# bramtoula/multi_robot_SLAM_separators

Hardware: AMD Instinct MI355X
Metric: candidate keyframe-pair verifications/sec (NetVLAD NN + ORB match + RANSAC) @1/2/4/8 GPU (higher is better)
Workload: dtype u8+f16+f32+f64

## Files before the change

multi_robot_slam_separators_amd/csrc/k_match.hip:

```cpp
#include "sf_internal.hpp"
#include <type_traits>

namespace {

__device__ __forceinline__ uint32_t bcnt_acc(uint32_t x, uint32_t acc) {
  uint32_t r;
  asm("v_bcnt_u32_b32 %0, %1, %2" : "=v"(r) : "v"(x), "v"(acc));
  return r;
}

template <int W, int NQ>
__device__ __forceinline__ void knn2_scan(const uint32_t* __restrict__ dF, int Kf, const uint32_t (&q)[NQ][W],
                                          uint32_t (&k1)[NQ], uint32_t (&k2)[NQ]) {
#pragma unroll 4
  for (int f = 0; f < Kf; ++f) {
    const uint32_t* r = dF + (size_t)f * W;
    uint32_t x[W];
#pragma unroll
    for (int c = 0; c < W; ++c) x[c] = r[c];
#pragma unroll
    for (int j = 0; j < NQ; ++j) {
      uint32_t d = 0;
#pragma unroll
      for (int c = 0; c < W; ++c) d = bcnt_acc(x[c] ^ q[j][c], d);
      const uint32_t key = (d << 16) | (uint32_t)f;
      k2[j] = min(max(key, k1[j]), k2[j]);
      k1[j] = min(k1[j], key);
    }
  }
}

template <int W>
__device__ __forceinline__ void knn2_scan_l2(const uint32_t* __restrict__ dF, int Kf, const uint32_t (&q)[W], float& d1,
                                             float& d2, int& i1) {
#pragma unroll 1
  for (int f = 0; f < Kf; ++f) {
    const uint32_t* r = dF + (size_t)f * W;
    float s = 0.f;
#pragma unroll
    for (int c = 0; c < W; ++c) {
      const float d = __uint_as_float(q[c]) - __uint_as_float(r[c]);
      s = s + d * d;
    }
    if (s < d1) { d2 = d1; d1 = s; i1 = f; }
    else if (s < d2) { d2 = s; }
  }
}

template <int W>
__device__ __forceinline__ void knn2_scan_l2_halves(const uint32_t* __restrict__ dF, int Kf,
                                                    const uint32_t* __restrict__ qrow, float& d1, float& d2, int& i1) {
  static_assert(W == 128, "two halves of 64 dimensions");
  constexpr int H = 64, FB = 16;
#pragma unroll 1
  for (int f0 = 0; f0 < Kf; f0 += FB) {
    float s[FB];
#pragma unroll
    for (int j = 0; j < FB; ++j) s[j] = 0.f;
#pragma unroll 1
    for (int half = 0; half < 2; ++half) {
      uint32_t q[H];
      {
        const uint4* p = reinterpret_cast<const uint4*>(qrow + half * H);
#pragma unroll
        for (int c = 0; c < H / 4; ++c) {
          const uint4 v = p[c];
          q[4 * c] = v.x; q[4 * c + 1] = v.y; q[4 * c + 2] = v.z; q[4 * c + 3] = v.w;
        }
      }
#pragma unroll
      for (int j = 0; j < FB; ++j) {
        if (f0 + j < Kf) {
          const uint32_t* r = dF + (size_t)(f0 + j) * W + half * H;
          float a = s[j];
#pragma unroll
          for (int c = 0; c < H; ++c) {
            const float d = __uint_as_float(q[c]) - __uint_as_float(r[c]);
            a = a + d * d;
          }
          s[j] = a;
        }
      }
    }
#pragma unroll
    for (int j = 0; j < FB; ++j) {
      if (f0 + j < Kf) {
        if (s[j] < d1) { d2 = d1; d1 = s[j]; i1 = f0 + j; }
        else if (s[j] < d2) { d2 = s[j]; }
      }
    }
  }
}

template <int W>
__device__ __forceinline__ void load_desc(const uint32_t* __restrict__ base, int row, bool valid, uint32_t (&q)[W]) {
  const uint4* p = reinterpret_cast<const uint4*>(base + (size_t)(valid ? row : 0) * W);
#pragma unroll
  for (int c = 0; c < W / 4; ++c) {
    uint4 v = p[c];
    q[4 * c + 0] = v.x; q[4 * c + 1] = v.y; q[4 * c + 2] = v.z; q[4 * c + 3] = v.w;
  }
}

template <int W, int NQ, int NT, bool L2 = false>
__global__ void __launch_bounds__(NT)
k_match_global(StoreView st, const int32_t* __restrict__ pair_from, const int32_t* __restrict__ pair_to,
               float nndr, int min_inliers, int est, uint32_t* __restrict__ corr, CorrHeader* __restrict__ hdr,
               PassState* __restrict__ pass, int32_t* __restrict__ list, int32_t* __restrict__ counter) {
  extern __shared__ __attribute__((aligned(16))) int smem[];
  constexpr int NW = NT / 64;
  const int pair = blockIdx.x;
  const int tid = threadIdx.x;
  const int lane = tid & 63, wave = tid >> 6;
  const int kcap = st.kcap;
  const int sF = pair_from[pair], sT = pair_to[pair];
  if ((unsigned)sF >= (unsigned)st.n_slots || (unsigned)sT >= (unsigned)st.n_slots) {
    if (tid == 0) {
      CorrHeader h = {0, 0, 0, 0};
      hdr[pair] = h;
      PassState ps;
#pragma unroll
      for (int i = 0; i < 12; ++i) ps.T[i] = 0.f;
      ps.var = 1.0; ps.var_ang = 1.0; ps.is_null = 1; ps.inliers = 0; ps.matches = 0; ps.pad = 0;
      pass[pair] = ps;
    }
    return;
  }
  const int4 mF = st.meta[sF], mT = st.meta[sT];
  const int Kf = mF.x, Kt = mT.x;
  const uint32_t* dF = st.desc + (size_t)sF * kcap * W;
  const uint32_t* dT = st.desc + (size_t)sT * kcap * W;

  int* cnt = smem;
  int* owner = smem + kcap;
  int* misc = smem + 2 * kcap;

  for (int i = tid; i < Kf; i += NT) cnt[i] = 0;
  if (tid < 16) misc[tid] = 0;
  __syncthreads();

  int rejected = 0;
  if constexpr (L2) {
    static_assert(!L2 || NQ == 1, "one resident float row per lane");
    if (Kf > 0) {
      for (int base = 0; base < Kt; base += NT) {
        const int t = base + tid;
        float d1 = __int_as_float(0x7F800000), d2 = __int_as_float(0x7F800000);
        int i1 = -1;
        if constexpr (W > 64) {
          if (Kt - base - (tid & ~63) > 0)
            knn2_scan_l2_halves<W>(dF, Kf, dT + (size_t)(t < Kt ? t : 0) * W, d1, d2, i1);
        } else {
          uint32_t q[W];
          load_desc<W>(dT, t, t < Kt, q);
          if (Kt - base - (tid & ~63) > 0)
            knn2_scan_l2<W>(dF, Kf, q, d1, d2, i1);
        }
        if (t < Kt) {
          const bool acc = (Kf >= 2) && i1 >= 0 && !(d1 > nndr * d2);
          if (acc) {
            atomicAdd(&cnt[i1], 1);
            owner[i1] = t;
          } else {
            ++rejected;
          }
        }
      }
    }
  } else
  if (Kf > 0) {
    for (int base = 0; base < Kt; base += NQ * NT) {
      uint32_t q[NQ][W], k1[NQ], k2[NQ];
#pragma unroll
      for (int j = 0; j < NQ; ++j) {
        const int t = base + j * NT + tid;
        load_desc<W>(dT, t, t < Kt, q[j]);
        k1[j] = 0xFFFFFFFFu;
        k2[j] = 0xFFFFFFFFu;
      }
      const int wave_rows = Kt - base - (tid & ~63);
      const int groups = wave_rows <= 0 ? 0 : min(NQ, (wave_rows + NT - 1) / NT);
      if (groups == NQ) {
        knn2_scan<W, NQ>(dF, Kf, q, k1, k2);
      } else if (groups > 0) {
#pragma unroll
        for (int j = 0; j < NQ; ++j) {
          if (j < groups) {
            uint32_t qq[1][W], a1[1] = {0xFFFFFFFFu}, a2[1] = {0xFFFFFFFFu};
#pragma unroll
            for (int c = 0; c < W; ++c) qq[0][c] = q[j][c];
            knn2_scan<W, 1>(dF, Kf, qq, a1, a2);
            k1[j] = a1[0];
            k2[j] = a2[0];
          }
        }
      }
#pragma unroll
      for (int j = 0; j < NQ; ++j) {
        const int t = base + j * NT + tid;
        if (t < Kt) {
          const bool acc = (Kf >= 2) && !((float)(k1[j] >> 16) > nndr * (float)(k2[j] >> 16));
          if (acc) {
            const int f = (int)(k1[j] & 0xFFFFu);
            atomicAdd(&cnt[f], 1);
            owner[f] = t;
          } else {
            ++rejected;
          }
        }
      }
    }
  }
  for (int off = 32; off >= 1; off >>= 1) rejected += __shfl_xor(rejected, off);
  if (lane == 0 && rejected) atomicAdd(&misc[0], rejected);
  __syncthreads();

  uint32_t* out = corr + (size_t)pair * kcap;
  int running = 0;
  for (int base = 0; base < Kf; base += NT) {
    const int f = base + tid;
    const bool flag = (f < Kf) && (cnt[f] == 1);
    const unsigned long long bal = __ballot(flag);
    const int before = __popcll(bal & ((1ull << lane) - 1ull));
    if (lane == 0) misc[4 + wave] = __popcll(bal);
    __syncthreads();
    int woff = 0, total = 0;
#pragma unroll
    for (int w = 0; w < NW; ++w) {
      int c = misc[4 + w];
      if (w < wave) woff += c;
      total += c;
    }
    if (flag) out[running + woff + before] = (uint32_t)f | ((uint32_t)owner[f] << 16);
    running += total;
    __syncthreads();
  }
  const int n_corr = running;

  const int unique_to = (Kf > 0 && Kt > 0) ? misc[0] + n_corr : 0;
  const int words_from = (Kf > 0 && mF.y > 0) ? Kf : 0;
  const int words_to = (mT.y > 0) ? unique_to : 0;
  const bool motion = est == 0 ? (unique_to > 0 && words_from >= min_inliers && words_to >= min_inliers)
                    : est == 1 ? (unique_to > 0 && words_from >= min_inliers && unique_to >= min_inliers)
                               : (est == 3 && unique_to > 0 && ((words_from >= min_inliers && unique_to >= min_inliers) ||
                                                                (words_to >= min_inliers && Kf >= min_inliers)));
  const bool survivor = est == 3 ? (motion && n_corr > 0) : (motion && n_corr >= min_inliers && n_corr >= (est == 0 ? 3 : 4));
  if (motion && !survivor) {
    const float* xF = st.xyz + (size_t)sF * kcap * 3;
    const float* xT = st.xyz + (size_t)sT * kcap * 3;
    for (int i = tid; i < n_corr; i += NT) {
      uint32_t c = out[i];
      const float* a = xF + 3 * (c & 0xFFFFu);
      const float* b = xT + 3 * (c >> 16);
      bool ok = isfinite(a[0]) && isfinite(a[1]) && isfinite(a[2]);
      if (est == 0)
        ok = ok && isfinite(b[0]) && isfinite(b[1]) && isfinite(b[2]) && (a[0] != 0.f || a[1] != 0.f || a[2] != 0.f) &&
             (b[0] != 0.f || b[1] != 0.f || b[2] != 0.f);
      if (ok) atomicAdd(&misc[2], 1);
    }
    __syncthreads();
  }
  if (tid == 0) {
    CorrHeader h;
    h.n_corr = n_corr;
    h.words_from = words_from;
    h.words_to = words_to;
    h.words_to_2d = unique_to;
    hdr[pair] = h;
    PassState ps;
#pragma unroll
    for (int i = 0; i < 12; ++i) ps.T[i] = 0.f;
    ps.var = 1.0; ps.var_ang = 1.0;
    ps.is_null = 1;
    ps.inliers = 0;
    ps.matches = (motion && !survivor) ? misc[2] : 0;
    ps.pad = 0;
    pass[pair] = ps;
    if (survivor) {
      int pos = atomicAdd(counter, 1);
      list[pos] = pair;
    }
  }
}

__device__ __forceinline__ uint32_t min_u16(uint32_t a, uint32_t b) {
  uint32_t r;
  asm("v_min_u16 %0, %1, %2" : "=v"(r) : "v"(a), "v"(b));
  return r;
}
__device__ __forceinline__ uint32_t max_u16(uint32_t a, uint32_t b) {
  uint32_t r;
  asm("v_max_u16 %0, %1, %2" : "=v"(r) : "v"(a), "v"(b));
  return r;
}

constexpr int MATCH_CH = 16;

template <int W, int NQ>
__device__ __forceinline__ void knn2_step_lds(const uint32_t* fromD, int f, const uint32_t (&q)[NQ][W],
                                              uint32_t (&d1)[NQ], uint32_t (&d2)[NQ]) {
  const uint4* r = reinterpret_cast<const uint4*>(fromD + (size_t)f * W);
  uint32_t x[W];
#pragma unroll
  for (int c = 0; c < W / 4; ++c) {
    const uint4 v = r[c];
    x[4 * c] = v.x; x[4 * c + 1] = v.y; x[4 * c + 2] = v.z; x[4 * c + 3] = v.w;
  }
#pragma unroll
  for (int j = 0; j < NQ; ++j) {
    uint32_t d = 0;
#pragma unroll
    for (int c = 0; c < W; ++c) d = bcnt_acc(x[c] ^ q[j][c], d);
    d2[j] = min_u16(d2[j], max_u16(d, d1[j]));
    d1[j] = min_u16(d1[j], d);
  }
}

template <int W, int NQ>
__device__ __forceinline__ void knn2_scan_lds(const uint32_t* fromD, int Kf, const uint32_t (&q)[NQ][W],
                                              uint32_t (&d1)[NQ], uint32_t (&d2)[NQ], uint32_t (&chunk)[NQ]) {
  int c0 = 0;
  for (; c0 + MATCH_CH <= Kf; c0 += MATCH_CH) {
    uint32_t prev[NQ];
#pragma unroll
    for (int j = 0; j < NQ; ++j) prev[j] = d1[j];
#pragma unroll 4
    for (int u = 0; u < MATCH_CH; ++u) knn2_step_lds<W, NQ>(fromD, c0 + u, q, d1, d2);
#pragma unroll
    for (int j = 0; j < NQ; ++j) chunk[j] = ((d1[j] & 0xFFFFu) != (prev[j] & 0xFFFFu)) ? (uint32_t)c0 : chunk[j];
  }
  if (c0 < Kf) {
    uint32_t prev[NQ];
#pragma unroll
    for (int j = 0; j < NQ; ++j) prev[j] = d1[j];
    for (int f = c0; f < Kf; ++f) knn2_step_lds<W, NQ>(fromD, f, q, d1, d2);
#pragma unroll
    for (int j = 0; j < NQ; ++j) chunk[j] = ((d1[j] & 0xFFFFu) != (prev[j] & 0xFFFFu)) ? (uint32_t)c0 : chunk[j];
  }
}

typedef int mf_v8i __attribute__((ext_vector_type(8)));
typedef float mf_v16f __attribute__((ext_vector_type(16)));
constexpr float MF_FR = 1.f / 2048.f;
constexpr int MF_MAX_ROWS = 2048;

__device__ __forceinline__ mf_v8i fp4_spread_from(uint32_t x, uint32_t m88, uint32_t c22) {
  mf_v8i o = {0, 0, 0, 0, 0, 0, 0, 0};
  o[0] = (int)((x & m88) | c22);
  o[1] = (int)(x & 0x44444444u);
  o[2] = (int)(x & 0x22222222u);
  o[3] = (int)(x & 0x11111111u);
  return o;
}
__device__ __forceinline__ mf_v8i fp4_spread_to(uint32_t y, uint32_t m88, uint32_t c22) {
  mf_v8i o = {0, 0, 0, 0, 0, 0, 0, 0};
  const uint32_t n = ~y;
  o[0] = (int)((y & m88) | c22);
  o[1] = (int)(((n << 1) & m88) | c22);
  o[2] = (int)(((n << 2) & m88) | 0x44444444u);
  o[3] = (int)(((n << 3) & m88) | 0x66666666u);
  return o;
}

static inline size_t sf_match_lds_bytes(int kcap, int w) {
  const int behind = 2 * kcap + 16;
  return (size_t)(kcap * w + (behind > 32 * w ? behind : 32 * w)) * sizeof(int);
}

template <int KS>
__device__ __forceinline__ void load_raw(const uint32_t* p, uint32_t (&raw)[KS]) {
#pragma unroll
  for (int c = 0; c < KS / 4; ++c) {
    const uint4 v = reinterpret_cast<const uint4*>(p)[c];
    raw[4 * c] = v.x; raw[4 * c + 1] = v.y; raw[4 * c + 2] = v.z; raw[4 * c + 3] = v.w;
  }
}

__device__ __forceinline__ void top2_update16(const mf_v16f& v, float& b, float& s) {
  const float x0 = __builtin_amdgcn_fmed3f(b, v[0], v[1]);
  float ta, tb;
  asm("v_max3_f32 %0, %0, %4, %5\n\t"
      "v_med3_f32 %2, %0, %6, %7\n\t"
      "v_max3_f32 %0, %0, %6, %7\n\t"
      "v_max3_f32 %1, %1, %20, %2\n\t"
      "v_med3_f32 %2, %0, %8, %9\n\t"
      "v_max3_f32 %0, %0, %8, %9\n\t"
      "v_med3_f32 %3, %0, %10, %11\n\t"
      "v_max3_f32 %0, %0, %10, %11\n\t"
      "v_max3_f32 %1, %1, %2, %3\n\t"
      "v_med3_f32 %2, %0, %12, %13\n\t"
      "v_max3_f32 %0, %0, %12, %13\n\t"
      "v_med3_f32 %3, %0, %14, %15\n\t"
      "v_max3_f32 %0, %0, %14, %15\n\t"
      "v_max3_f32 %1, %1, %2, %3\n\t"
      "v_med3_f32 %2, %0, %16, %17\n\t"
      "v_max3_f32 %0, %0, %16, %17\n\t"
      "v_med3_f32 %3, %0, %18, %19\n\t"
      "v_max3_f32 %0, %0, %18, %19\n\t"
      "v_max3_f32 %1, %1, %2, %3"
      : "+v"(b), "+v"(s), "=&v"(ta), "=&v"(tb)
      : "v"(v[0]), "v"(v[1]), "v"(v[2]), "v"(v[3]), "v"(v[4]), "v"(v[5]), "v"(v[6]), "v"(v[7]), "v"(v[8]), "v"(v[9]),
        "v"(v[10]), "v"(v[11]), "v"(v[12]), "v"(v[13]), "v"(v[14]), "v"(v[15]), "v"(x0));
}

template <int W, int NTL, bool TAIL>
__device__ __forceinline__ void knn2_mfma_tile(const uint32_t* fromD, int Kf, int mt, int r, int h,
                                               const mf_v8i (&Bf)[NTL][W / 2], const float (&cin)[16],
                                               float (&b)[NTL], float (&s)[NTL], uint32_t m88, uint32_t c22,
                                               uint32_t (&raw)[W / 2], const uint32_t*& nxt) {
  constexpr int KS = W / 2;
  mf_v16f c0;
#pragma unroll
  for (int i = 0; i < 16; ++i) c0[i] = cin[i];
  mf_v8i Af[KS];
#pragma unroll
  for (int k = 0; k < KS; ++k) Af[k] = fp4_spread_from(raw[k], m88, c22);
  if (!TAIL) {
    nxt += 32 * W;
    load_raw<KS>(nxt, raw);
  }
#pragma unroll
  for (int j = 0; j < NTL; ++j) {
    b[j] += 32.f * MF_FR;
    s[j] += 32.f * MF_FR;
  }
#pragma unroll
  for (int j = 0; j < NTL; ++j) {
    mf_v16f acc = __builtin_amdgcn_mfma_scale_f32_32x32x64_f8f6f4(Af[0], Bf[j][0], c0, 4, 4, 0, 0, 0, 0);
#pragma unroll
    for (int k = 1; k < KS; ++k)
      acc = __builtin_amdgcn_mfma_scale_f32_32x32x64_f8f6f4(Af[k], Bf[j][k], acc, 4, 4, 0, 0, 0, 0);
    if (TAIL) {
      const int left = Kf - mt * 32 - 4 * h;
#pragma unroll
      for (int i = 0; i < 16; ++i) acc[i] = ((i & 3) + 8 * (i >> 2) < left) ? acc[i] : -INFINITY;
    }
    top2_update16(acc, b[j], s[j]);
  }
}

template <int W, int NTL>
struct MfB {
  mf_v8i Bf[NTL][W / 2];
  int tsum[NTL];
};

template <int W, int NTL>
__device__ __forceinline__ void mf_load_b(const uint32_t* __restrict__ dT, int Kt, const int (&tile)[NTL], int lane,
                                          MfB<W, NTL>& B) {
  constexpr int KS = W / 2;
  const int r = lane & 31, h = lane >> 5;
  uint32_t m88, c22;
  asm volatile("v_mov_b32 %0, 0x88888888" : "=v"(m88));
  asm volatile("v_mov_b32 %0, 0x22222222" : "=v"(c22));
#pragma unroll
  for (int j = 0; j < NTL; ++j) {
    const int t = tile[j] * 32 + r;
    uint32_t raw[KS];
#pragma unroll
    for (int k = 0; k < KS; ++k) raw[k] = 0;
    if (t < Kt) load_raw<KS>(dT + (size_t)t * W + KS * h, raw);
    int p = 0;
#pragma unroll
    for (int k = 0; k < KS; ++k) {
      B.Bf[j][k] = fp4_spread_to(raw[k], m88, c22);
      p += __popc(raw[k] & 0x77777777u);
    }
    p += __shfl_xor(p, 32);
    B.tsum[j] = 24 * W - 2 * p;
  }
}

typedef int mf_v4i __attribute__((ext_vector_type(4)));

__device__ __forceinline__ void mf_pipe_half1(mf_v16f& acc, const mf_v4i& a0, const mf_v4i& a1, const mf_v4i& a2,
                                              const mf_v4i& a3, const mf_v4i& b0, const mf_v4i& b1, const mf_v16f& cin,
                                              const mf_v16f& old, float& b, float& s, float& x0, float& ta, float& tb) {
  asm volatile(
      "s_nop 1\n\t"
      "v_mfma_f32_32x32x64_f8f6f4 %[acc], %[a0], %[b0], %[cin] cbsz:4 blgp:4\n\t"
      "v_add_f32 %[b], 0x3c800000, %[b]\n\t"
      "v_add_f32 %[s], 0x3c800000, %[s]\n\t"
      "s_nop 1\n\t"
      "v_med3_f32 %[x0], %[b], %[o0], %[o1]\n\t"
      "v_max3_f32 %[b], %[b], %[o0], %[o1]\n\t"
      "v_mfma_f32_32x32x64_f8f6f4 %[acc], %[a1], %[b1], %[acc] cbsz:4 blgp:4\n\t"
      "v_med3_f32 %[ta], %[b], %[o2], %[o3]\n\t"
      "v_max3_f32 %[b], %[b], %[o2], %[o3]\n\t"
      "v_max3_f32 %[s], %[s], %[x0], %[ta]\n\t"
      "v_med3_f32 %[ta], %[b], %[o4], %[o5]\n\t"
      "v_max3_f32 %[b], %[b], %[o4], %[o5]\n\t"
      "v_med3_f32 %[tb], %[b], %[o6], %[o7]"
      : [acc] "=&v"(acc), [b] "+v"(b), [s] "+v"(s), [x0] "=&v"(x0), [ta] "=&v"(ta), [tb] "=&v"(tb)
      : [a0] "v"(a0), [a1] "v"(a1), "v"(a2), "v"(a3), [b0] "v"(b0), [b1] "v"(b1), [cin] "v"(cin), [o0] "v"(old[0]),
        [o1] "v"(old[1]), [o2] "v"(old[2]), [o3] "v"(old[3]), [o4] "v"(old[4]), [o5] "v"(old[5]), [o6] "v"(old[6]),
        [o7] "v"(old[7]));
}
__device__ __forceinline__ void mf_pipe_half2(mf_v16f& acc, const mf_v4i& a2, const mf_v4i& a3, const mf_v4i& b2,
                                              const mf_v4i& b3, const mf_v16f& old, float& b, float& s, float& ta,
                                              float& tb) {
  float x0;
  asm volatile(
      "v_mfma_f32_32x32x64_f8f6f4 %[acc], %[a2], %[b2], %[acc] cbsz:4 blgp:4\n\t"
      "v_max3_f32 %[b], %[b], %[o6], %[o7]\n\t"
      "v_max3_f32 %[s], %[s], %[ta], %[tb]\n\t"
      "v_med3_f32 %[x0], %[b], %[o8], %[o9]\n\t"
      "v_max3_f32 %[b], %[b], %[o8], %[o9]\n\t"
      "v_med3_f32 %[ta], %[b], %[o10], %[o11]\n\t"
      "v_max3_f32 %[b], %[b], %[o10], %[o11]\n\t"
      "v_mfma_f32_32x32x64_f8f6f4 %[acc], %[a3], %[b3], %[acc] cbsz:4 blgp:4\n\t"
      "v_max3_f32 %[s], %[s], %[x0], %[ta]\n\t"
      "v_med3_f32 %[ta], %[b], %[o12], %[o13]\n\t"
      "v_max3_f32 %[b], %[b], %[o12], %[o13]\n\t"
      "v_med3_f32 %[tb], %[b], %[o14], %[o15]\n\t"
      "v_max3_f32 %[b], %[b], %[o14], %[o15]\n\t"
      "v_max3_f32 %[s], %[s], %[ta], %[tb]"
      : [acc] "+v"(acc), [b] "+v"(b), [s] "+v"(s), [x0] "=&v"(x0), [ta] "+v"(ta), [tb] "+v"(tb)
      : [a2] "v"(a2), [a3] "v"(a3), [b2] "v"(b2), [b3] "v"(b3), [o6] "v"(old[6]), [o7] "v"(old[7]), [o8] "v"(old[8]),
        [o9] "v"(old[9]), [o10] "v"(old[10]), [o11] "v"(old[11]), [o12] "v"(old[12]), [o13] "v"(old[13]),
        [o14] "v"(old[14]), [o15] "v"(old[15]));
}
__device__ __forceinline__ void mf_pipe_drain(const mf_v16f& old, float& b, float& s) {
  float x0, ta, tb;
  asm volatile(
      "s_nop 11\n\t"
      "v_add_f32 %[b], 0x3c800000, %[b]\n\t"
      "v_add_f32 %[s], 0x3c800000, %[s]\n\t"
      "v_med3_f32 %[x0], %[b], %[o0], %[o1]\n\t"
      "v_max3_f32 %[b], %[b], %[o0], %[o1]\n\t"
      "v_med3_f32 %[ta], %[b], %[o2], %[o3]\n\t"
      "v_max3_f32 %[b], %[b], %[o2], %[o3]\n\t"
      "v_max3_f32 %[s], %[s], %[x0], %[ta]\n\t"
      "v_med3_f32 %[ta], %[b], %[o4], %[o5]\n\t"
      "v_max3_f32 %[b], %[b], %[o4], %[o5]\n\t"
      "v_med3_f32 %[tb], %[b], %[o6], %[o7]\n\t"
      "v_max3_f32 %[b], %[b], %[o6], %[o7]\n\t"
      "v_max3_f32 %[s], %[s], %[ta], %[tb]\n\t"
      "v_med3_f32 %[x0], %[b], %[o8], %[o9]\n\t"
      "v_max3_f32 %[b], %[b], %[o8], %[o9]\n\t"
      "v_med3_f32 %[ta], %[b], %[o10], %[o11]\n\t"
      "v_max3_f32 %[b], %[b], %[o10], %[o11]\n\t"
      "v_max3_f32 %[s], %[s], %[x0], %[ta]\n\t"
      "v_med3_f32 %[ta], %[b], %[o12], %[o13]\n\t"
      "v_max3_f32 %[b], %[b], %[o12], %[o13]\n\t"
      "v_med3_f32 %[tb], %[b], %[o14], %[o15]\n\t"
      "v_max3_f32 %[b], %[b], %[o14], %[o15]\n\t"
      "v_max3_f32 %[s], %[s], %[ta], %[tb]"
      : [b] "+v"(b), [s] "+v"(s), [x0] "=&v"(x0), [ta] "=&v"(ta), [tb] "=&v"(tb)
      : [o0] "v"(old[0]), [o1] "v"(old[1]), [o2] "v"(old[2]), [o3] "v"(old[3]), [o4] "v"(old[4]), [o5] "v"(old[5]),
        [o6] "v"(old[6]), [o7] "v"(old[7]), [o8] "v"(old[8]), [o9] "v"(old[9]), [o10] "v"(old[10]), [o11] "v"(old[11]),
        [o12] "v"(old[12]), [o13] "v"(old[13]), [o14] "v"(old[14]), [o15] "v"(old[15]));
}

template <int NTL>
__device__ __forceinline__ void mf_scan_full_tiles_pipe(const uint32_t* fromD, int n_full, const MfB<8, NTL>& B,
                                                        const float (&cin)[16], float (&b)[NTL], float (&s)[NTL],
                                                        uint32_t m88, uint32_t c22, uint32_t (&raw)[4],
                                                        const uint32_t*& nxt) {
  static_assert(NTL == 2 || NTL == 4, "tiles alternate between two accumulator tuples");
  if (n_full <= 0) return;
  mf_v4i B4[NTL][4];
#pragma unroll
  for (int j = 0; j < NTL; ++j) {
#pragma unroll
    for (int k = 0; k < 4; ++k) B4[j][k] = mf_v4i{B.Bf[j][k][0], B.Bf[j][k][1], B.Bf[j][k][2], B.Bf[j][k][3]};
  }
  mf_v16f c0, acc0, acc1;
#pragma unroll
  for (int i = 0; i < 16; ++i) { c0[i] = cin[i]; acc1[i] = -INFINITY; }
  for (int mt = 0; mt < n_full; ++mt) {
    mf_v4i A4[4];
#pragma unroll
    for (int k = 0; k < 4; ++k) {
      const mf_v8i a = fp4_spread_from(raw[k], m88, c22);
      A4[k] = mf_v4i{a[0], a[1], a[2], a[3]};
    }
    nxt += 32 * 8;
    load_raw<4>(nxt, raw);
#pragma unroll
    for (int j = 0; j < NTL; j += 2) {
      constexpr int JP = NTL - 1;
      float x0, ta, tb;
      const int jp = j == 0 ? JP : j - 1;
      mf_pipe_half1(acc0, A4[0], A4[1], A4[2], A4[3], B4[j][0], B4[j][1], c0, acc1, b[jp], s[jp], x0, ta, tb);
      mf_pipe_half2(acc0, A4[2], A4[3], B4[j][2], B4[j][3], acc1, b[jp], s[jp], ta, tb);
      mf_pipe_half1(acc1, A4[0], A4[1], A4[2], A4[3], B4[j + 1][0], B4[j + 1][1], c0, acc0, b[j], s[j], x0, ta, tb);
      mf_pipe_half2(acc1, A4[2], A4[3], B4[j + 1][2], B4[j + 1][3], acc0, b[j], s[j], ta, tb);
    }
  }
  mf_pipe_drain(acc1, b[NTL - 1], s[NTL - 1]);
}

template <int W, int NTL, bool PIPE = false>
__device__ __forceinline__ void mf_scan(const uint32_t* fromD, int Kf, const MfB<W, NTL>& B, int lane,
                                        uint32_t (&d1)[NTL], uint32_t (&d2)[NTL], int (&idx)[NTL]) {
  constexpr int KS = W / 2;
  const int r = lane & 31, h = lane >> 5;
  uint32_t m88, c22;
  asm volatile("v_mov_b32 %0, 0x88888888" : "=v"(m88));
  asm volatile("v_mov_b32 %0, 0x22222222" : "=v"(c22));
  float cin[16], b[NTL], s[NTL];
#pragma unroll
  for (int i = 0; i < 16; ++i) cin[i] = -(float)((i & 3) + 8 * (i >> 2) + 4 * h) * MF_FR;
#pragma unroll
  for (int j = 0; j < NTL; ++j) { b[j] = -INFINITY; s[j] = -INFINITY; }
  const int n_full = Kf >> 5;
  uint32_t raw[KS];
  load_raw<KS>(fromD + (size_t)min(r, Kf - 1) * W + KS * h, raw);
  const uint32_t* nxt = fromD + (size_t)r * W + KS * h;
  if constexpr (PIPE && W == 8 && (NTL == 2 || NTL == 4)) {
    mf_scan_full_tiles_pipe<NTL>(fromD, n_full, B, cin, b, s, m88, c22, raw, nxt);
  } else {
    for (int mt = 0; mt < n_full; ++mt) knn2_mfma_tile<W, NTL, false>(fromD, Kf, mt, r, h, B.Bf, cin, b, s, m88, c22, raw, nxt);
  }
  if (Kf & 31) knn2_mfma_tile<W, NTL, true>(fromD, Kf, n_full, r, h, B.Bf, cin, b, s, m88, c22, raw, nxt);
  const float org = (float)(32 * (((Kf + 31) >> 5) - 1)) * MF_FR;
#pragma unroll
  for (int j = 0; j < NTL; ++j) {
    const float ob = __shfl_xor(b[j], 32), os = __shfl_xor(s[j], 32);
    const float nb = fmaxf(b[j], ob) - org;
    const float ns = fmaxf(fminf(b[j], ob), fmaxf(s[j], os)) - org;
    const float dot1 = 2.f * ceilf(nb * 0.5f), dot2 = 2.f * ceilf(ns * 0.5f);
    idx[j] = (int)((dot1 - nb) * 2048.f);
    d1[j] = (uint32_t)((32 * W - B.tsum[j] - (int)dot1) >> 1);
    d2[j] = ns == -INFINITY ? 0xFFFFu : (uint32_t)((32 * W - B.tsum[j] - (int)dot2) >> 1);
  }
}

template <int W, int NTL, bool PIPE = false>
__device__ __forceinline__ void knn2_mfma(const uint32_t* fromD, int Kf, const uint32_t* __restrict__ dT, int Kt,
                                          const int (&tile)[NTL], int lane, uint32_t (&d1)[NTL], uint32_t (&d2)[NTL],
                                          int (&idx)[NTL]) {
  MfB<W, NTL> B;
  mf_load_b<W, NTL>(dT, Kt, tile, lane, B);
  mf_scan<W, NTL, PIPE>(fromD, Kf, B, lane, d1, d2, idx);
}

template <int W, int NQ, int NT, int MF_NTL = 2, bool MF_PIPE = false>
__device__ __forceinline__ bool match_v2_body(const StoreView& st, int pair, int sF, int sT, float nndr, int min_inliers,
                                              int est, uint32_t* out, CorrHeader& hdr_out, PassState& pass_out,
                                              int32_t* __restrict__ list, int32_t* __restrict__ counter, int* smem,
                                              unsigned long long* trace_row = nullptr) {
  constexpr int NW = NT / 64;
  const int tid = threadIdx.x;
  const int lane = tid & 63, wave = tid >> 6;
  const int kcap = st.kcap;
  if ((unsigned)sF >= (unsigned)st.n_slots || (unsigned)sT >= (unsigned)st.n_slots) {
    if (tid == 0) {
      CorrHeader h = {0, 0, 0, 0};
      hdr_out = h;
      PassState ps;
#pragma unroll
      for (int i = 0; i < 12; ++i) ps.T[i] = 0.f;
      ps.var = 1.0; ps.var_ang = 1.0; ps.is_null = 1; ps.inliers = 0; ps.matches = 0; ps.pad = 0;
      pass_out = ps;
    }
    return false;
  }
  const int4 mF = st.meta[sF], mT = st.meta[sT];
  const int Kf = mF.x, Kt = mT.x;
  const uint32_t* dF = st.desc + (size_t)sF * kcap * W;
  const uint32_t* dT = st.desc + (size_t)sT * kcap * W;

  uint32_t* fromD = reinterpret_cast<uint32_t*>(smem);
  int* cnt = smem + kcap * W;
  int* owner = cnt + kcap;
  int* misc = owner + kcap;

  {
    const uint4* src = reinterpret_cast<const uint4*>(dF);
    uint4* dst = reinterpret_cast<uint4*>(fromD);
    for (int i = tid; i < Kf * (W / 4); i += NT) dst[i] = src[i];
  }
  for (int i = tid; i < Kf; i += NT) cnt[i] = 0;
  if (tid < 16) misc[tid] = 0;
  __syncthreads();
  SF_TRACE_ROW_MARK(trace_row, 32);

  int rejected = 0;
  if constexpr (NQ == 0) {
    if (Kf > 0) {
      constexpr int NTL = W == 8 ? MF_NTL : 1;
      const int n_nt = (Kt + 31) >> 5;
      auto group = [&](auto g, int t0) {
        constexpr int G = decltype(g)::value;
        int tl[G], f[G];
        uint32_t a1[G], a2[G];
#pragma unroll
        for (int j = 0; j < G; ++j) tl[j] = t0 + j * NW;
        knn2_mfma<W, G, MF_PIPE>(fromD, Kf, dT, Kt, tl, lane, a1, a2, f);
#pragma unroll
        for (int j = 0; j < G; ++j) {
          const int t = tl[j] * 32 + lane;
          if (lane < 32 && t < Kt) {
            const bool acc = (Kf >= 2) && !((float)a1[j] > nndr * (float)a2[j]);
            if (acc) {
              atomicAdd(&cnt[f[j]], 1);
              owner[f[j]] = t;
            } else {
              ++rejected;
            }
          }
        }
      };
      for (int t0 = wave; t0 < n_nt; t0 += NW * NTL) {
        const int avail = (n_nt - t0 + NW - 1) / NW;
        if (NTL >= 4 && avail >= 3) group(std::integral_constant<int, 4>{}, t0);
        else if (NTL >= 2 && avail >= 2) group(std::integral_constant<int, 2>{}, t0);
        else group(std::integral_constant<int, 1>{}, t0);
      }
    }
  } else if (Kf > 0) {
    for (int base = 0; base < Kt; base += NQ * NT) {

      uint32_t q[NQ][W], d1[NQ], d2[NQ], chunk[NQ];
#pragma unroll
      for (int j = 0; j < NQ; ++j) {
        const int t = base + j * NT + tid;
        load_desc<W>(dT, t, t < Kt, q[j]);
        d1[j] = 0xFFFFu;
        d2[j] = 0xFFFFu;
        chunk[j] = 0;
      }
      const int wave_rows = Kt - base - (tid & ~63);
      const int groups = wave_rows <= 0 ? 0 : min(NQ, (wave_rows + NT - 1) / NT);
      if (groups == NQ) {
        knn2_scan_lds<W, NQ>(fromD, Kf, q, d1, d2, chunk);
      } else if (groups > 0) {
#pragma unroll
        for (int j = 0; j < NQ; ++j) {
          if (j < groups) {
            uint32_t qq[1][W], a1[1] = {0xFFFFu}, a2[1] = {0xFFFFu}, ch[1] = {0};
#pragma unroll
            for (int c = 0; c < W; ++c) qq[0][c] = q[j][c];
            knn2_scan_lds<W, 1>(fromD, Kf, qq, a1, a2, ch);
            d1[j] = a1[0]; d2[j] = a2[0]; chunk[j] = ch[0];
          }
        }
      }
#pragma unroll
      for (int j = 0; j < NQ; ++j) {
        const int t = base + j * NT + tid;
        if (t < Kt) {
          const uint32_t b1 = d1[j] & 0xFFFFu, b2 = d2[j] & 0xFFFFu;
          const bool acc = (Kf >= 2) && !((float)b1 > nndr * (float)b2);
          if (acc) {
            int f = (int)chunk[j];
            const int fend = min(f + MATCH_CH, Kf);
            for (; f < fend; ++f) {
              const uint32_t* r = fromD + (size_t)f * W;
              uint32_t d = 0;
#pragma unroll
              for (int c = 0; c < W; ++c) d += __popc(r[c] ^ q[j][c]);
              if (d == b1) break;
            }
            atomicAdd(&cnt[f], 1);
            owner[f] = t;
          } else {
            ++rejected;
          }
        }
      }
    }
  }
  for (int off = 32; off >= 1; off >>= 1) rejected += __shfl_xor(rejected, off);
  if (lane == 0 && rejected) atomicAdd(&misc[0], rejected);
  SF_TRACE_ROW_MARK(trace_row, 33);
  __syncthreads();
  SF_TRACE_ROW_MARK(trace_row, 34);

  int running = 0;
  for (int base = 0; base < Kf; base += NT) {
    const int f = base + tid;
    const bool flag = (f < Kf) && (cnt[f] == 1);
    const unsigned long long bal = __ballot(flag);
    const int before = __popcll(bal & ((1ull << lane) - 1ull));
    if (lane == 0) misc[4 + wave] = __popcll(bal);
    __syncthreads();
    int woff = 0, total = 0;
#pragma unroll
    for (int w = 0; w < NW; ++w) {
      int c = misc[4 + w];
      if (w < wave) woff += c;
      total += c;
    }
    if (flag) out[running + woff + before] = (uint32_t)f | ((uint32_t)owner[f] << 16);
    running += total;
    __syncthreads();
  }
  const int n_corr = running;
  SF_TRACE_ROW_MARK(trace_row, 35);

  const int unique_to = (Kf > 0 && Kt > 0) ? misc[0] + n_corr : 0;
  const int words_from = (Kf > 0 && mF.y > 0) ? Kf : 0;
  const int words_to = (mT.y > 0) ? unique_to : 0;
  const bool motion = est == 0 ? (unique_to > 0 && words_from >= min_inliers && words_to >= min_inliers)
                    : est == 1 ? (unique_to > 0 && words_from >= min_inliers && unique_to >= min_inliers)
                               : (est == 3 && unique_to > 0 && ((words_from >= min_inliers && unique_to >= min_inliers) ||
                                                                (words_to >= min_inliers && Kf >= min_inliers)));
  const bool survivor = est == 3 ? (motion && n_corr > 0) : (motion && n_corr >= min_inliers && n_corr >= (est == 0 ? 3 : 4));
  if (motion && !survivor) {
    const float* xF = st.xyz + (size_t)sF * kcap * 3;
    const float* xT = st.xyz + (size_t)sT * kcap * 3;
    for (int i = tid; i < n_corr; i += NT) {
      uint32_t c = out[i];
      const float* a = xF + 3 * (c & 0xFFFFu);
      const float* b = xT + 3 * (c >> 16);
      bool ok = isfinite(a[0]) && isfinite(a[1]) && isfinite(a[2]);
      if (est == 0)
        ok = ok && isfinite(b[0]) && isfinite(b[1]) && isfinite(b[2]) && (a[0] != 0.f || a[1] != 0.f || a[2] != 0.f) &&
             (b[0] != 0.f || b[1] != 0.f || b[2] != 0.f);
      if (ok) atomicAdd(&misc[2], 1);
    }
    __syncthreads();
  }
  if (tid == 0) {
    CorrHeader h;
    h.n_corr = n_corr;
    h.words_from = words_from;
    h.words_to = words_to;
    h.words_to_2d = unique_to;
    hdr_out = h;
    PassState ps;
#pragma unroll
    for (int i = 0; i < 12; ++i) ps.T[i] = 0.f;
    ps.var = 1.0; ps.var_ang = 1.0;
    ps.is_null = 1;
    ps.inliers = 0;
    ps.matches = (motion && !survivor) ? misc[2] : 0;
    ps.pad = 0;
    pass_out = ps;
    if (survivor && list) {
      int pos = atomicAdd(counter, 1);
      list[pos] = pair;
    }
  }
  return survivor;
}

template <int W, int NQ, int NT>
__global__ void __launch_bounds__(NT)
k_match_global_v2(StoreView st, const int32_t* __restrict__ pair_from, const int32_t* __restrict__ pair_to,
                  float nndr, int min_inliers, int est, uint32_t* __restrict__ corr, CorrHeader* __restrict__ hdr,
                  PassState* __restrict__ pass, int32_t* __restrict__ list, int32_t* __restrict__ counter) {
  extern __shared__ __attribute__((aligned(16))) int smem[];
  const int pair = (int)blockIdx.x;
  match_v2_body<W, NQ, NT>(st, pair, pair_from[pair], pair_to[pair], nndr, min_inliers, est, corr + (size_t)pair * st.kcap,
                           hdr[pair], pass[pair], list, counter, smem);
}

template <int W, int NT>
__global__ void __launch_bounds__(NT, 2)
k_match_global_mf(StoreView st, const int32_t* __restrict__ pair_from, const int32_t* __restrict__ pair_to,
                  float nndr, int min_inliers, int est, uint32_t* __restrict__ corr, CorrHeader* __restrict__ hdr,
                  PassState* __restrict__ pass, int32_t* __restrict__ list, int32_t* __restrict__ counter) {
  extern __shared__ __attribute__((aligned(16))) int smem[];
  const int pair = (int)blockIdx.x;
  match_v2_body<W, 0, NT, 4>(st, pair, pair_from[pair], pair_to[pair], nndr, min_inliers, est,
                             corr + (size_t)pair * st.kcap, hdr[pair], pass[pair], list, counter, smem);
}

template <int W, int NQ, int NT>
void launch_match_v2(sf_context* c, StoreView st, const int32_t* d_from, const int32_t* d_to, int n) {
  size_t lds = sf_match_lds_bytes(st.kcap, W);
  if (const char* v = getenv("SF_MATCH_LDS_PAD")) lds += (size_t)atoi(v);
  int32_t* counters = (int32_t*)c->w->counters.p;
  if constexpr (NQ == 0)
    hipLaunchKernelGGL((k_match_global_mf<W, NT>), dim3(n), dim3(NT), lds, c->stream, st, d_from, d_to,
                       c->dparams.nndr, c->dparams.min_inliers, sf_est_mode(c), (uint32_t*)c->w->corr1.p,
                       (CorrHeader*)c->w->hdr1.p, (PassState*)c->w->pass1.p, (int32_t*)c->w->list1.p, counters + 0);
  else
    hipLaunchKernelGGL((k_match_global_v2<W, NQ, NT>), dim3(n), dim3(NT), lds, c->stream, st, d_from, d_to,
                       c->dparams.nndr, c->dparams.min_inliers, sf_est_mode(c), (uint32_t*)c->w->corr1.p,
                       (CorrHeader*)c->w->hdr1.p, (PassState*)c->w->pass1.p, (int32_t*)c->w->list1.p, counters + 0);
}

template <int W, int NQ, int NT>
void launch_match(sf_context* c, StoreView st, const int32_t* d_from, const int32_t* d_to, int n) {
  const size_t lds = (size_t)(2 * st.kcap + 16) * sizeof(int);
  int32_t* counters = (int32_t*)c->w->counters.p;
  hipLaunchKernelGGL((k_match_global<W, NQ, NT>), dim3(n), dim3(NT), lds, c->stream, st, d_from, d_to,
                     c->dparams.nndr, c->dparams.min_inliers, sf_est_mode(c), (uint32_t*)c->w->corr1.p, (CorrHeader*)c->w->hdr1.p,
                     (PassState*)c->w->pass1.p, (int32_t*)c->w->list1.p, counters + 0);
}

template <int W>
void launch_match_l2(sf_context* c, StoreView st, const int32_t* d_from, const int32_t* d_to, int n) {
  const size_t lds = (size_t)(2 * st.kcap + 16) * sizeof(int);
  int32_t* counters = (int32_t*)c->w->counters.p;
  hipLaunchKernelGGL((k_match_global<W, 1, 256, true>), dim3(n), dim3(256), lds, c->stream, st, d_from, d_to,
                     c->dparams.nndr, c->dparams.min_inliers, sf_est_mode(c), (uint32_t*)c->w->corr1.p, (CorrHeader*)c->w->hdr1.p,
                     (PassState*)c->w->pass1.p, (int32_t*)c->w->list1.p, counters + 0);
}

}

int sf_launch_match_global(sf_context* c, StoreView st, const int32_t* d_from, const int32_t* d_to, int n) {
  if (n <= 0) return SF_OK;
  if (c->params.desc_type == 1) {
    sf_prof_begin(c, SF_K_MATCH);
    if (st.w == 64) launch_match_l2<64>(c, st, d_from, d_to, n);
    else launch_match_l2<128>(c, st, d_from, d_to, n);
    sf_prof_end(c, SF_K_MATCH);
    SF_HIP(c, hipGetLastError());
    return SF_OK;
  }
  int variant = c->match_variant;
  if (variant == 0) {
    const size_t lds_v2 = sf_match_lds_bytes(st.kcap, st.w);
    variant = lds_v2 <= 64 * 1024 ? (c->match_mfma && st.kcap <= MF_MAX_ROWS ? 10256 : 12256) : 2256;
  }
  sf_prof_begin(c, SF_K_MATCH);
#define SF_CASE(NQ_, NT_)                                                        \
  case NQ_ * 1000 + NT_:                                                         \
    if (st.w == 8) launch_match<8, NQ_, NT_>(c, st, d_from, d_to, n);            \
    else launch_match<16, NQ_, NT_>(c, st, d_from, d_to, n);                     \
    break;
  switch (variant) {
    SF_CASE(1, 256)
    SF_CASE(2, 256)
    SF_CASE(4, 128)
    SF_CASE(2, 128)
    SF_CASE(4, 256)
    SF_CASE(8, 64)
    SF_CASE(4, 64)
#define SF_CASE2(NQ_, NT_)                                                          \
  case 10000 + NQ_ * 1000 + NT_:                                                    \
    if (st.w == 8) launch_match_v2<8, NQ_, NT_>(c, st, d_from, d_to, n);            \
    else launch_match_v2<16, NQ_, NT_>(c, st, d_from, d_to, n);                     \
    break;
    SF_CASE2(0, 256)
    SF_CASE2(2, 256)
    SF_CASE2(1, 256)
    SF_CASE2(4, 128)
    SF_CASE2(2, 128)
#undef SF_CASE2
    default:
      sf_prof_end(c, SF_K_MATCH);
      return sf_fail(c, SF_EINVAL, "unknown match kernel variant %d", variant);
  }
#undef SF_CASE
  sf_prof_end(c, SF_K_MATCH);
  SF_HIP(c, hipGetLastError());
  return SF_OK;
}
```

Before: 23.22 million.

## Pack two column tiles per wave via permlane32 swap in MFMA kNN epilogue

The epilogue that merged the two half-wave top-2 results now uses permlane32_swap to pair tiles, so that lanes 0-31 finalize one tile and lanes 32-63 finalize the next. This halves the per-tile shuffles and epilogue ALU work, and both wave halves now do useful accept/reject work instead of only lanes below 32. The tail tile in the pipelined path is now handled by masking the bias input rather than falling back to the non-pipelined tile routine. The distance and index arithmetic is also refolded into fma/ceil form with precomputed constants, which adds some risk of numeric or index mismatch.

Result: faster. 23.74 million (median of 6 runs) (+2.2%).

```diff
diff --git a/multi_robot_slam_separators_amd/csrc/k_match.hip b/multi_robot_slam_separators_amd/csrc/k_match.hip
--- a/multi_robot_slam_separators_amd/csrc/k_match.hip
+++ b/multi_robot_slam_separators_amd/csrc/k_match.hip
@@ -439,10 +439,19 @@
   }
 }
 
+template <int NTL>
+constexpr int mf_pairs() { return (NTL + 1) / 2; }
+
+__device__ __forceinline__ void mf_merge_halves(uint32_t& x, uint32_t& y) {
+  const auto r = __builtin_amdgcn_permlane32_swap(x, y, false, false);
+  x = r[0];
+  y = r[1];
+}
+
 template <int W, int NTL>
 struct MfB {
   mf_v8i Bf[NTL][W / 2];
-  int tsum[NTL];
+  int ch[mf_pairs<NTL>()];
 };
 
 template <int W, int NTL>
@@ -453,6 +462,7 @@
   uint32_t m88, c22;
   asm volatile("v_mov_b32 %0, 0x88888888" : "=v"(m88));
   asm volatile("v_mov_b32 %0, 0x22222222" : "=v"(c22));
+  uint32_t p[NTL];
 #pragma unroll
   for (int j = 0; j < NTL; ++j) {
     const int t = tile[j] * 32 + r;
@@ -460,14 +470,19 @@
 #pragma unroll
     for (int k = 0; k < KS; ++k) raw[k] = 0;
     if (t < Kt) load_raw<KS>(dT + (size_t)t * W + KS * h, raw);
-    int p = 0;
+    p[j] = 0;
 #pragma unroll
     for (int k = 0; k < KS; ++k) {
       B.Bf[j][k] = fp4_spread_to(raw[k], m88, c22);
-      p += __popc(raw[k] & 0x77777777u);
-    }
-    p += __shfl_xor(p, 32);
-    B.tsum[j] = 24 * W - 2 * p;
+      p[j] += __popc(raw[k] & 0x77777777u);
+    }
+  }
+#pragma unroll
+  for (int q = 0; q < mf_pairs<NTL>(); ++q) {
+    uint32_t x = p[2 * q], y = p[2 * q + 1 < NTL ? 2 * q + 1 : 2 * q];
+    mf_merge_halves(x, y);
+    B.ch[q] = (int)(x + y) + 4 * W;
+    asm volatile("" : "+v"(B.ch[q]));
   }
 }
 
@@ -552,48 +567,92 @@
         [o12] "v"(old[12]), [o13] "v"(old[13]), [o14] "v"(old[14]), [o15] "v"(old[15]));
 }
 
-template <int NTL>
-__device__ __forceinline__ void mf_scan_full_tiles_pipe(const uint32_t* fromD, int n_full, const MfB<8, NTL>& B,
-                                                        const float (&cin)[16], float (&b)[NTL], float (&s)[NTL],
-                                                        uint32_t m88, uint32_t c22, uint32_t (&raw)[4],
-                                                        const uint32_t*& nxt) {
-  static_assert(NTL == 2 || NTL == 4, "tiles alternate between two accumulator tuples");
-  if (n_full <= 0) return;
-  mf_v4i B4[NTL][4];
-#pragma unroll
-  for (int j = 0; j < NTL; ++j) {
-#pragma unroll
-    for (int k = 0; k < 4; ++k) B4[j][k] = mf_v4i{B.Bf[j][k][0], B.Bf[j][k][1], B.Bf[j][k][2], B.Bf[j][k][3]};
-  }
-  mf_v16f c0, acc0, acc1;
-#pragma unroll
-  for (int i = 0; i < 16; ++i) { c0[i] = cin[i]; acc1[i] = -INFINITY; }
-  for (int mt = 0; mt < n_full; ++mt) {
-    mf_v4i A4[4];
-#pragma unroll
-    for (int k = 0; k < 4; ++k) {
-      const mf_v8i a = fp4_spread_from(raw[k], m88, c22);
-      A4[k] = mf_v4i{a[0], a[1], a[2], a[3]};
-    }
+template <int NTL, bool NEXT>
+__device__ __forceinline__ void mf_pipe_tile(const mf_v4i (&B4)[NTL][4], const mf_v16f& c0, mf_v16f& acc0,
+                                             mf_v16f& acc1, float (&b)[NTL], float (&s)[NTL], uint32_t m88, uint32_t c22,
+                                             uint32_t (&raw)[4], const uint32_t*& nxt) {
+  mf_v4i A4[4];
+#pragma unroll
+  for (int k = 0; k < 4; ++k) {
+    const mf_v8i a = fp4_spread_from(raw[k], m88, c22);
+    A4[k] = mf_v4i{a[0], a[1], a[2], a[3]};
+  }
+  if (NEXT) {
     nxt += 32 * 8;
     load_raw<4>(nxt, raw);
-#pragma unroll
-    for (int j = 0; j < NTL; j += 2) {
-      constexpr int JP = NTL - 1;
-      float x0, ta, tb;
-      const int jp = j == 0 ? JP : j - 1;
-      mf_pipe_half1(acc0, A4[0], A4[1], A4[2], A4[3], B4[j][0], B4[j][1], c0, acc1, b[jp], s[jp], x0, ta, tb);
-      mf_pipe_half2(acc0, A4[2], A4[3], B4[j][2], B4[j][3], acc1, b[jp], s[jp], ta, tb);
-      mf_pipe_half1(acc1, A4[0], A4[1], A4[2], A4[3], B4[j + 1][0], B4[j + 1][1], c0, acc0, b[j], s[j], x0, ta, tb);
-      mf_pipe_half2(acc1, A4[2], A4[3], B4[j + 1][2], B4[j + 1][3], acc0, b[j], s[j], ta, tb);
-    }
+  }
+#pragma unroll
+  for (int j = 0; j < NTL; j += 2) {
+    constexpr int JP = NTL - 1;
+    float x0, ta, tb;
+    const int jp = j == 0 ? JP : j - 1;
+    mf_pipe_half1(acc0, A4[0], A4[1], A4[2], A4[3], B4[j][0], B4[j][1], c0, acc1, b[jp], s[jp], x0, ta, tb);
+    mf_pipe_half2(acc0, A4[2], A4[3], B4[j][2], B4[j][3], acc1, b[jp], s[jp], ta, tb);
+    mf_pipe_half1(acc1, A4[0], A4[1], A4[2], A4[3], B4[j + 1][0], B4[j + 1][1], c0, acc0, b[j], s[j], x0, ta, tb);
+    mf_pipe_half2(acc1, A4[2], A4[3], B4[j + 1][2], B4[j + 1][3], acc0, b[j], s[j], ta, tb);
+  }
+}
+
+template <int NTL>
+__device__ __forceinline__ void mf_scan_tiles_pipe(int Kf, const MfB<8, NTL>& B, const float (&cin)[16],
+                                                   float (&b)[NTL], float (&s)[NTL], uint32_t m88, uint32_t c22,
+                                                   uint32_t (&raw)[4], const uint32_t*& nxt) {
+  static_assert(NTL == 2 || NTL == 4, "tiles alternate between two accumulator tuples");
+  mf_v4i B4[NTL][4];
+#pragma unroll
+  for (int j = 0; j < NTL; ++j) {
+#pragma unroll
+    for (int k = 0; k < 4; ++k) B4[j][k] = mf_v4i{B.Bf[j][k][0], B.Bf[j][k][1], B.Bf[j][k][2], B.Bf[j][k][3]};
+  }
+  mf_v16f c0, acc0, acc1;
+#pragma unroll
+  for (int i = 0; i < 16; ++i) { c0[i] = cin[i]; acc1[i] = -INFINITY; }
+  const int n_full = Kf >> 5;
+  for (int mt = 0; mt < n_full; ++mt) mf_pipe_tile<NTL, true>(B4, c0, acc0, acc1, b, s, m88, c22, raw, nxt);
+  if (Kf & 31) {
+    int kr = Kf & 31;
+    asm volatile("" : "+s"(kr));
+    const float lim = -(float)kr * MF_FR;
+#pragma unroll
+    for (int i = 0; i < 16; ++i) c0[i] = c0[i] > lim ? c0[i] : -INFINITY;
+    mf_pipe_tile<NTL, false>(B4, c0, acc0, acc1, b, s, m88, c22, raw, nxt);
   }
   mf_pipe_drain(acc1, b[NTL - 1], s[NTL - 1]);
+}
+
+__device__ __forceinline__ int mf_cvt_i32(float x) {
+  int r;
+  asm("v_cvt_i32_f32 %0, %1" : "=v"(r) : "v"(x));
+  return r;
+}
+__device__ __forceinline__ float mf_max(float a, float b) {
+  float r;
+  asm("v_max_f32 %0, %1, %2" : "=v"(r) : "v"(a), "v"(b));
+  return r;
+}
+__device__ __forceinline__ float mf_min(float a, float b) {
+  float r;
+  asm("v_min_f32 %0, %1, %2" : "=v"(r) : "v"(a), "v"(b));
+  return r;
+}
+__device__ __forceinline__ float mf_max3(float a, float b, float c) {
+  float r;
+  asm("v_max3_f32 %0, %1, %2, %3" : "=v"(r) : "v"(a), "v"(b), "v"(c));
+  return r;
+}
+template <int NTL>
+__device__ __forceinline__ void mf_swap_wait(float (&b)[NTL], float (&s)[NTL]) {
+  static_assert(NTL == 1 || NTL == 2 || NTL == 4, "column tiles per scan");
+  if constexpr (NTL == 1) asm volatile("s_nop 1" : "+v"(b[0]), "+v"(s[0]));
+  else if constexpr (NTL == 2) asm volatile("s_nop 1" : "+v"(b[0]), "+v"(s[0]), "+v"(b[1]), "+v"(s[1]));
+  else
+    asm volatile("s_nop 1" : "+v"(b[0]), "+v"(s[0]), "+v"(b[1]), "+v"(s[1]), "+v"(b[2]), "+v"(s[2]), "+v"(b[3]), "+v"(s[3]));
 }
 
 template <int W, int NTL, bool PIPE = false>
 __device__ __forceinline__ void mf_scan(const uint32_t* fromD, int Kf, const MfB<W, NTL>& B, int lane,
-                                        uint32_t (&d1)[NTL], uint32_t (&d2)[NTL], int (&idx)[NTL]) {
+                                        uint32_t (&d1)[mf_pairs<NTL>()], uint32_t (&d2)[mf_pairs<NTL>()],
+                                        int (&idx)[mf_pairs<NTL>()]) {
   constexpr int KS = W / 2;
   const int r = lane & 31, h = lane >> 5;
   uint32_t m88, c22;
@@ -609,28 +668,34 @@
   load_raw<KS>(fromD + (size_t)min(r, Kf - 1) * W + KS * h, raw);
   const uint32_t* nxt = fromD + (size_t)r * W + KS * h;
   if constexpr (PIPE && W == 8 && (NTL == 2 || NTL == 4)) {
-    mf_scan_full_tiles_pipe<NTL>(fromD, n_full, B, cin, b, s, m88, c22, raw, nxt);
+    mf_scan_tiles_pipe<NTL>(Kf, B, cin, b, s, m88, c22, raw, nxt);
   } else {
     for (int mt = 0; mt < n_full; ++mt) knn2_mfma_tile<W, NTL, false>(fromD, Kf, mt, r, h, B.Bf, cin, b, s, m88, c22, raw, nxt);
-  }
-  if (Kf & 31) knn2_mfma_tile<W, NTL, true>(fromD, Kf, n_full, r, h, B.Bf, cin, b, s, m88, c22, raw, nxt);
-  const float org = (float)(32 * (((Kf + 31) >> 5) - 1)) * MF_FR;
-#pragma unroll
-  for (int j = 0; j < NTL; ++j) {
-    const float ob = __shfl_xor(b[j], 32), os = __shfl_xor(s[j], 32);
-    const float nb = fmaxf(b[j], ob) - org;
-    const float ns = fmaxf(fminf(b[j], ob), fmaxf(s[j], os)) - org;
-    const float dot1 = 2.f * ceilf(nb * 0.5f), dot2 = 2.f * ceilf(ns * 0.5f);
-    idx[j] = (int)((dot1 - nb) * 2048.f);
-    d1[j] = (uint32_t)((32 * W - B.tsum[j] - (int)dot1) >> 1);
-    d2[j] = ns == -INFINITY ? 0xFFFFu : (uint32_t)((32 * W - B.tsum[j] - (int)dot2) >> 1);
+    if (Kf & 31) knn2_mfma_tile<W, NTL, true>(fromD, Kf, n_full, r, h, B.Bf, cin, b, s, m88, c22, raw, nxt);
+  }
+  const int orow = 32 * (((Kf + 31) >> 5) - 1);
+  const float horg = -0.5f * ((float)orow * MF_FR), org2k = (float)orow;
+  mf_swap_wait<NTL>(b, s);
+#pragma unroll
+  for (int q = 0; q < mf_pairs<NTL>(); ++q) {
+    const int j0 = 2 * q, j1 = 2 * q + 1 < NTL ? 2 * q + 1 : 2 * q;
+    uint32_t xb = __float_as_uint(b[j0]), yb = __float_as_uint(b[j1]);
+    uint32_t xs = __float_as_uint(s[j0]), ys = __float_as_uint(s[j1]);
+    mf_merge_halves(xb, yb);
+    mf_merge_halves(xs, ys);
+    const float x = __uint_as_float(xb), y = __uint_as_float(yb);
+    const float nb = mf_max(x, y), ns = mf_max3(mf_min(x, y), __uint_as_float(xs), __uint_as_float(ys));
+    const float h1 = ceilf(__builtin_fmaf(nb, 0.5f, horg)), h2 = ceilf(__builtin_fmaf(ns, 0.5f, horg));
+    idx[q] = (int)__builtin_fmaf(h1, 4096.f, __builtin_fmaf(nb, -2048.f, org2k));
+    d1[q] = (uint32_t)(B.ch[q] - (int)h1);
+    d2[q] = min((uint32_t)B.ch[q] - (uint32_t)mf_cvt_i32(h2), 0xFFFFu);
   }
 }
 
 template <int W, int NTL, bool PIPE = false>
 __device__ __forceinline__ void knn2_mfma(const uint32_t* fromD, int Kf, const uint32_t* __restrict__ dT, int Kt,
-                                          const int (&tile)[NTL], int lane, uint32_t (&d1)[NTL], uint32_t (&d2)[NTL],
-                                          int (&idx)[NTL]) {
+                                          const int (&tile)[NTL], int lane, uint32_t (&d1)[mf_pairs<NTL>()],
+                                          uint32_t (&d2)[mf_pairs<NTL>()], int (&idx)[mf_pairs<NTL>()]) {
   MfB<W, NTL> B;
   mf_load_b<W, NTL>(dT, Kt, tile, lane, B);
   mf_scan<W, NTL, PIPE>(fromD, Kf, B, lane, d1, d2, idx);
@@ -683,20 +748,21 @@
       constexpr int NTL = W == 8 ? MF_NTL : 1;
       const int n_nt = (Kt + 31) >> 5;
       auto group = [&](auto g, int t0) {
-        constexpr int G = decltype(g)::value;
-        int tl[G], f[G];
-        uint32_t a1[G], a2[G];
+        constexpr int G = decltype(g)::value, NP = mf_pairs<G>();
+        int tl[G], f[NP];
+        uint32_t a1[NP], a2[NP];
 #pragma unroll
         for (int j = 0; j < G; ++j) tl[j] = t0 + j * NW;
         knn2_mfma<W, G, MF_PIPE>(fromD, Kf, dT, Kt, tl, lane, a1, a2, f);
 #pragma unroll
-        for (int j = 0; j < G; ++j) {
-          const int t = tl[j] * 32 + lane;
-          if (lane < 32 && t < Kt) {
-            const bool acc = (Kf >= 2) && !((float)a1[j] > nndr * (float)a2[j]);
+        for (int q = 0; q < NP; ++q) {
+          const bool hi = lane >= 32;
+          const int t = (hi ? tl[2 * q + 1 < G ? 2 * q + 1 : 2 * q] : tl[2 * q]) * 32 + (lane & 31);
+          if ((!hi || 2 * q + 1 < G) && t < Kt) {
+            const bool acc = (Kf >= 2) && !((float)a1[q] > nndr * (float)a2[q]);
             if (acc) {
-              atomicAdd(&cnt[f[j]], 1);
-              owner[f[j]] = t;
+              atomicAdd(&cnt[f[q]], 1);
+              owner[f[q]] = t;
             } else {
               ++rejected;
             }
```
